# neggles/neurosis

Hardware: AMD Instinct MI355X
Metric: train images/sec (node) SDXL 1024^2 (higher is better)
Workload: dtype bf16

## Files before the change

### neurosis_amd/csrc/conv_wgrad_halo.h

```cpp
#pragma once


typedef __attribute__((address_space(3))) char* wh_lds;
typedef __attribute__((address_space(3))) short4_t* wh_lds4;

__device__ __forceinline__ int wh_swz_x(int slot) { return (((slot >> 1) & 1) << 2) | ((slot >> 2) & 3); }
__device__ __forceinline__ int wh_swz_dy(int px) { return ((px & 3) << 2) | ((px >> 2) & 3); }

__device__ __forceinline__ bf16x8_t wh_read(wh_lds lo, wh_lds hi) {
  const short4_t a = __builtin_amdgcn_ds_read_tr16_b64_v4i16((wh_lds4)lo);
  const short4_t b = __builtin_amdgcn_ds_read_tr16_b64_v4i16((wh_lds4)hi);
  short8_t r;
  r[0] = a[0]; r[1] = a[1]; r[2] = a[2]; r[3] = a[3];
  r[4] = b[0]; r[5] = b[1]; r[6] = b[2]; r[7] = b[3];
  return __builtin_bit_cast(bf16x8_t, r);
}

struct WhStager {
  int xd, xe, dd, de;
  int n, ty, tx;

  __device__ __forceinline__ void init(const NkGemmParams& p, int t, int txn, int tyn, int lane) {
    const int per_img = txn * tyn;
    n = t / per_img;
    const int rem = t - n * per_img;
    ty = rem / txn;
    tx = rem - ty * txn;
    const int l8 = lane >> 3, l16 = lane >> 4;
    xd = (lane & 7) ^ ((((l8 >> 1) & 1) << 2) | (l8 >> 2));
    xe = l8 * p.gb.C;
    dd = (lane & 15) ^ (l16 << 2);
    de = l16 * (int)p.lda;
  }
  __device__ __forceinline__ void issue(const NkGemmParams& p, char* stage, int txn, int tyn, int cb, int ib, int wave, int lane) {
    const NkGather& g = p.gb;
    const int h0 = ty * WH_TH, w0 = tx * WH_TW;
    const bf16_t* xo = p.B + (((long)n * g.H + h0 - 1) * g.W + (w0 - 1)) * g.C + ib * WH_BCI;
    const bf16_t* dyo = p.A + (((long)n * g.H + h0) * g.W + w0) * p.lda + cb * WH_BCO;
    const bf16_t* zp = (const bf16_t*)nk_zero_page;
    int l8 = lane >> 3, l16 = lane >> 4, xd_ = xd, xe_ = xe, dd_ = dd, de_ = de;
    asm volatile("" : "+v"(l8), "+v"(l16), "+v"(xd_), "+v"(xe_), "+v"(dd_), "+v"(de_));
#pragma unroll
    for (int i = 0; i < 8; ++i) {
      const int pc = wave + 8 * i;
      if (pc < 30) {
        const int hr = pc / 5, pg = pc - hr * 5;
        const bool row_ok = (unsigned)(h0 - 1 + hr) < (unsigned)g.H;
        const int slot = pg * 8 + l8;
        const bool v = row_ok && slot < WH_TW + 2 && (unsigned)(w0 - 1 + slot) < (unsigned)g.W;
        const int off = (hr * g.W + pg * 8) * g.C + xe_ + ((xd_ ^ ((pg & 1) << 1)) << 3);
        __builtin_amdgcn_global_load_lds((nk_gptr)(v ? xo + off : zp), (nk_lptr)(stage + (hr * WH_HS + pg * 8) * 128), 16, 0, 0);
      } else if (pc < 62) {
        const int q = pc - 30;
        const bool row_ok = h0 + (q >> 3) < g.H;
        const int chunk = dd_ ^ (q & 3);
        const bool v = row_ok && w0 + (q & 7) * 4 + l16 < g.W && cb * WH_BCO + chunk * 8 < p.M;
        const int off = ((q >> 3) * g.W + (q & 7) * 4) * (int)p.lda + de_ + (chunk << 3);
        __builtin_amdgcn_global_load_lds((nk_gptr)(v ? dyo + off : zp), (nk_lptr)(stage + WH_X_BYTES + q * 1024), 16, 0, 0);
      }
    }
    if (++tx == txn) { tx = 0; if (++ty == tyn) { ty = 0; ++n; } }
  }
};

template <int BIAS>
__global__ __launch_bounds__(512, 2) void nk_conv3x3_wgrad_halo_kernel(const NkGemmParams p) {
  extern __shared__ __attribute__((aligned(16))) char smem[];
  const int tid = threadIdx.x, lane = tid & 63;
  const int wave = __builtin_amdgcn_readfirstlane(tid >> 6);
  const int cs = wave & 3, is = wave >> 2;
  const NkGather& g = p.gb;
  const int Cin = g.C, Cout = p.M;
  const int nci = Cin / WH_BCI;
  const int nblk = ((Cout + WH_BCO - 1) / WH_BCO) * nci;
  const int blk = blockIdx.x % nblk, split = blockIdx.x / nblk;
  const int cb = blk / nci, ib = blk - cb * nci;
  const int txn = (g.W + WH_TW - 1) / WH_TW, tyn = (g.H + WH_TH - 1) / WH_TH;
  const int T = p.halo_nb * txn * tyn;
  const int t0 = split * p.ksplit_len, t1 = min(T, t0 + p.ksplit_len);

  float16_t acc[9];
#pragma unroll
  for (int t = 0; t < 9; ++t)
#pragma unroll
    for (int r = 0; r < 16; ++r) acc[t][r] = 0.f;
  float bsum = 0.f;

  const int h = lane >> 5, g1 = (lane >> 4) & 1, q4 = (lane & 15) >> 2, pp = lane & 3;
  unsigned xo[3][2], dyo[2];
#pragma unroll
  for (int j = 0; j < 2; ++j) {
#pragma unroll
    for (int a = 0; a < 3; ++a) {
      const int row = a + 4 * h + q4 + 8 * j;
      xo[a][j] = (unsigned)(row * 128 + (((4 * is + 2 * g1 + (pp >> 1)) ^ wh_swz_x(row)) << 4) + 8 * (pp & 1));
    }
    const int row = 4 * h + q4 + 8 * j;
    dyo[j] = (unsigned)(WH_X_BYTES + row * 256 + (((4 * cs + 2 * g1 + (pp >> 1)) ^ wh_swz_dy(row)) << 4) + 8 * (pp & 1));
  }
  const wh_lds sm = (wh_lds)smem;

  WhStager stg;
  stg.init(p, t0 < t1 ? t0 : 0, txn, tyn, lane);
  if (t0 < t1) stg.issue(p, smem, txn, tyn, cb, ib, wave, lane);
  for (int t = t0; t < t1; ++t) {
    const int st = (t - t0) & 1;
    asm volatile("s_waitcnt vmcnt(0)" ::: "memory");
    __syncthreads();
    if (t + 1 < t1) stg.issue(p, smem + (st ^ 1) * WH_STAGE, txn, tyn, cb, ib, wave, lane);
    const wh_lds base = sm + st * WH_STAGE;
#pragma unroll
    for (int kg = 0; kg < 8; ++kg) {
      const int r = kg >> 1, c = (kg & 1) * 16;
      const bf16x8_t af = wh_read(base + dyo[0] + kg * 4096, base + dyo[1] + kg * 4096);
      if constexpr (BIAS) {
        const short8_t raw = __builtin_bit_cast(short8_t, af);
#pragma unroll
        for (int e = 0; e < 8; ++e) bsum += bf2f((bf16_t)raw[e]);
      }
#pragma unroll
      for (int kh = 0; kh < 3; ++kh)
#pragma unroll
        for (int kw = 0; kw < 3; ++kw) {
          const int off = ((r + kh) * WH_HS + c) * 128;
          const bf16x8_t xf = wh_read(base + xo[kw][0] + off, base + xo[kw][1] + off);
          acc[kh * 3 + kw] = __builtin_amdgcn_mfma_f32_32x32x16_bf16(af, xf, acc[kh * 3 + kw], 0, 0, 0);
        }
    }
  }

  float* dw = (float*)p.C;
  const int ci = ib * WH_BCI + is * 32 + (lane & 31);
  const int co_base = cb * WH_BCO + cs * 32 + 4 * h;
  const bool atomic = gridDim.x > (unsigned)nblk || p.accumulate == 1;
#pragma unroll
  for (int t = 0; t < 9; ++t)
#pragma unroll
    for (int r = 0; r < 16; ++r) {
      const int co = co_base + (r & 3) + 8 * (r >> 2);
      if (co < Cout) {
        float* dst = dw + (long)co * p.ldc + t * Cin + ci;
        const float v = acc[t][r] * p.alpha;
        if (atomic) unsafeAtomicAdd(dst, v);
        else *dst = v;
      }
    }
  if constexpr (BIAS) {
    if (ib == 0 && is == 0) {
      bsum += __shfl_xor(bsum, 32);
      const int co = cb * WH_BCO + cs * 32 + (lane & 31);
      if (lane < 32 && co < Cout) {
        if (atomic) unsafeAtomicAdd(p.dbias + co, bsum * p.alpha);
        else p.dbias[co] = bsum * p.alpha;
      }
    }
  }
}
```

Baseline: 27.03.

## Spread halo wgrad DMA issue across MFMA steps and window LDS reads

Restructures the 3x3 conv weight-gradient halo kernel so that the next tile's global-to-LDS loads are issued one piece per k-group, interleaved with the MFMA work, instead of all at once after the barrier. The tile body now preloads a sliding window of input-halo fragments and dY fragments into registers, reading each halo row once rather than re-reading it for every kernel-row tap. DMA uses inline asm that sets m0 directly, and the last tile is peeled so the prefetch condition disappears from the loop. Optional timestamp instrumentation is added behind a macro. The extra register windows may raise VGPR pressure under the 512x2 launch bound.

```diff
diff --git a/neurosis_amd/csrc/conv_wgrad_halo.h b/neurosis_amd/csrc/conv_wgrad_halo.h
--- a/neurosis_amd/csrc/conv_wgrad_halo.h
+++ b/neurosis_amd/csrc/conv_wgrad_halo.h
@@ -14,6 +14,18 @@
   r[0] = a[0]; r[1] = a[1]; r[2] = a[2]; r[3] = a[3];
   r[4] = b[0]; r[5] = b[1]; r[6] = b[2]; r[7] = b[3];
   return __builtin_bit_cast(bf16x8_t, r);
+}
+
+#ifndef NK_WGH_ASM_DMA
+#define NK_WGH_ASM_DMA 1
+#endif
+__device__ __forceinline__ void wh_dma(const bf16_t* src, unsigned dst) {
+#if NK_WGH_ASM_DMA
+  unsigned keep;
+  asm volatile("s_mov_b32 %0, m0\n\ts_mov_b32 m0, %2\n\ts_nop 0\n\tglobal_load_lds_dwordx4 %1, off\n\ts_mov_b32 m0, %0" : "=&s"(keep) : "v"(src), "s"(dst) : "memory");
+#else
+  __builtin_amdgcn_global_load_lds((nk_gptr)src, (nk_lptr)(wh_lds)(unsigned long)dst, 16, 0, 0);
+#endif
 }
 
 struct WhStager {
@@ -32,36 +44,155 @@
     dd = (lane & 15) ^ (l16 << 2);
     de = l16 * (int)p.lda;
   }
-  __device__ __forceinline__ void issue(const NkGemmParams& p, char* stage, int txn, int tyn, int cb, int ib, int wave, int lane) {
+  __device__ __forceinline__ void piece(const NkGemmParams& p, unsigned stage, int cb, int ib, int wave, int lane, int i) const {
     const NkGather& g = p.gb;
     const int h0 = ty * WH_TH, w0 = tx * WH_TW;
-    const bf16_t* xo = p.B + (((long)n * g.H + h0 - 1) * g.W + (w0 - 1)) * g.C + ib * WH_BCI;
-    const bf16_t* dyo = p.A + (((long)n * g.H + h0) * g.W + w0) * p.lda + cb * WH_BCO;
     const bf16_t* zp = (const bf16_t*)nk_zero_page;
     int l8 = lane >> 3, l16 = lane >> 4, xd_ = xd, xe_ = xe, dd_ = dd, de_ = de;
-    asm volatile("" : "+v"(l8), "+v"(l16), "+v"(xd_), "+v"(xe_), "+v"(dd_), "+v"(de_));
+    if (i >= 4) {
+      asm volatile("" : "+v"(l8), "+v"(xd_), "+v"(xe_));
+      const bf16_t* xo = p.B + (((long)n * g.H + h0 - 1) * g.W + (w0 - 1)) * g.C + ib * WH_BCI;
+      const int pc = 8 * (i - 4) + (i == 7 && wave >= 6 ? wave - 2 : wave);
+      const int hr = pc / 5, pg = pc - hr * 5;
+      const bool row_ok = (unsigned)(h0 - 1 + hr) < (unsigned)g.H;
+      const int slot = pg * 8 + l8;
+      const bool v = row_ok && slot < WH_TW + 2 && (unsigned)(w0 - 1 + slot) < (unsigned)g.W;
+      const int off = (hr * g.W + pg * 8) * g.C + xe_ + ((xd_ ^ ((pg & 1) << 1)) << 3);
+      wh_dma(v ? xo + off : zp, stage + (hr * WH_HS + pg * 8) * 128);
+    } else {
+      asm volatile("" : "+v"(l16), "+v"(dd_), "+v"(de_));
+      const bf16_t* dyo = p.A + (((long)n * g.H + h0) * g.W + w0) * p.lda + cb * WH_BCO;
+      const int q = wave + 8 * i;
+      const bool row_ok = h0 + (q >> 3) < g.H;
+      const int chunk = dd_ ^ (q & 3);
+      const bool v = row_ok && w0 + (q & 7) * 4 + l16 < g.W && cb * WH_BCO + chunk * 8 < p.M;
+      const int off = ((q >> 3) * g.W + (q & 7) * 4) * (int)p.lda + de_ + (chunk << 3);
+      wh_dma(v ? dyo + off : zp, stage + WH_X_BYTES + q * 1024);
+    }
+  }
+  __device__ __forceinline__ void advance(int txn, int tyn) {
+    if (++tx == txn) { tx = 0; if (++ty == tyn) { ty = 0; ++n; } }
+  }
+  __device__ __forceinline__ void issue(const NkGemmParams& p, unsigned stage, int txn, int tyn, int cb, int ib, int wave, int lane) {
+#pragma unroll
+    for (int i = 0; i < 8; ++i) piece(p, stage, cb, ib, wave, lane, i);
+    advance(txn, tyn);
+  }
+};
+
+#ifndef NK_WGH_WINDOW
+#define NK_WGH_WINDOW 1
+#endif
+#ifndef NK_WGH_SPREAD
+#define NK_WGH_SPREAD 1
+#endif
+#ifdef NK_WGH_STAMPS
+#define WGH_SLOTS 20
+#define WGH_MAXWG 4096
+__device__ unsigned long long nk_wgh_stamp_buf[WGH_SLOTS * WGH_MAXWG];
+extern "C" int nk_debug_wgh_stamps(unsigned long long* host_out, int nwg) {
+  if (nwg < 0 || nwg > WGH_MAXWG) return 1;
+  return hipMemcpyFromSymbol(host_out, HIP_SYMBOL(nk_wgh_stamp_buf), (size_t)nwg * WGH_SLOTS * sizeof(unsigned long long)) == hipSuccess ? 0 : 1;
+}
+struct WghClock {
+  unsigned long long last;
+  unsigned sum[10];
+  __device__ __forceinline__ static unsigned long long now() {
+    unsigned long long t;
+    __builtin_amdgcn_sched_barrier(0);
+    asm volatile("s_memtime %0\n\ts_waitcnt lgkmcnt(0)" : "=s"(t) :: "memory");
+    __builtin_amdgcn_sched_barrier(0);
+    return t;
+  }
+  __device__ __forceinline__ void start() {
+#pragma unroll
+    for (int i = 0; i < 10; ++i) sum[i] = 0;
+    last = now();
+  }
+  __device__ __forceinline__ void lap(int i) { const unsigned long long t = now(); sum[i] += (unsigned)(t - last); last = t; }
+  __device__ __forceinline__ void skip() { last = now(); }
+};
+#else
+struct WghClock {
+  __device__ __forceinline__ void start() {}
+  __device__ __forceinline__ void lap(int) {}
+  __device__ __forceinline__ void skip() {}
+};
+#endif
+
+template <int BIAS, bool NEXT>
+__device__ __forceinline__ void wh_tile(float16_t (&acc)[9], float& bsum, const wh_lds base, const unsigned (&xo)[3][2], const unsigned (&dyo)[2],
+                                        const WhStager& stg, const NkGemmParams& p, unsigned nstage, int cb, int ib, int wave, int lane, WghClock& clk) {
+  if constexpr (NEXT && !NK_WGH_SPREAD) {
+#pragma unroll
+    for (int i = 0; i < 8; ++i) stg.piece(p, nstage, cb, ib, wave, lane, i);
+  }
+  clk.lap(1);
+  if constexpr (NK_WGH_WINDOW) {
+    bf16x8_t hx[2][WH_TH + 2][3];
+    bf16x8_t af[8];
+    af[0] = wh_read(base + dyo[0], base + dyo[1]);
+#pragma unroll
+    for (int hr = 0; hr < 2; ++hr)
+#pragma unroll
+      for (int kw = 0; kw < 3; ++kw) hx[0][hr][kw] = wh_read(base + xo[kw][0] + hr * WH_HS * 128, base + xo[kw][1] + hr * WH_HS * 128);
 #pragma unroll
     for (int i = 0; i < 8; ++i) {
-      const int pc = wave + 8 * i;
-      if (pc < 30) {
-        const int hr = pc / 5, pg = pc - hr * 5;
-        const bool row_ok = (unsigned)(h0 - 1 + hr) < (unsigned)g.H;
-        const int slot = pg * 8 + l8;
-        const bool v = row_ok && slot < WH_TW + 2 && (unsigned)(w0 - 1 + slot) < (unsigned)g.W;
-        const int off = (hr * g.W + pg * 8) * g.C + xe_ + ((xd_ ^ ((pg & 1) << 1)) << 3);
-        __builtin_amdgcn_global_load_lds((nk_gptr)(v ? xo + off : zp), (nk_lptr)(stage + (hr * WH_HS + pg * 8) * 128), 16, 0, 0);
-      } else if (pc < 62) {
-        const int q = pc - 30;
-        const bool row_ok = h0 + (q >> 3) < g.H;
-        const int chunk = dd_ ^ (q & 3);
-        const bool v = row_ok && w0 + (q & 7) * 4 + l16 < g.W && cb * WH_BCO + chunk * 8 < p.M;
-        const int off = ((q >> 3) * g.W + (q & 7) * 4) * (int)p.lda + de_ + (chunk << 3);
-        __builtin_amdgcn_global_load_lds((nk_gptr)(v ? dyo + off : zp), (nk_lptr)(stage + WH_X_BYTES + q * 1024), 16, 0, 0);
-      }
-    }
-    if (++tx == txn) { tx = 0; if (++ty == tyn) { ty = 0; ++n; } }
-  }
-};
+      const int ch = i >> 2, r = i & 3;
+#pragma unroll
+      for (int kw = 0; kw < 3; ++kw) {
+        const int off = ((r + 2) * WH_HS + ch * 16) * 128;
+        hx[ch][r + 2][kw] = wh_read(base + xo[kw][0] + off, base + xo[kw][1] + off);
+      }
+      if (i < 7) {
+        const int kg = 2 * ((i + 1) & 3) + ((i + 1) >> 2);
+        af[i + 1] = wh_read(base + dyo[0] + kg * 4096, base + dyo[1] + kg * 4096);
+      }
+      if (i == 3) {
+#pragma unroll
+        for (int hr = 0; hr < 2; ++hr)
+#pragma unroll
+          for (int kw = 0; kw < 3; ++kw) {
+            const int off = (hr * WH_HS + 16) * 128;
+            hx[1][hr][kw] = wh_read(base + xo[kw][0] + off, base + xo[kw][1] + off);
+          }
+      }
+      if constexpr (NEXT && NK_WGH_SPREAD) stg.piece(p, nstage, cb, ib, wave, lane, i);
+      if constexpr (BIAS) {
+        const short8_t raw = __builtin_bit_cast(short8_t, af[i]);
+#pragma unroll
+        for (int e = 0; e < 8; ++e) bsum += bf2f((bf16_t)raw[e]);
+      }
+#pragma unroll
+      for (int kh = 0; kh < 3; ++kh)
+#pragma unroll
+        for (int kw = 0; kw < 3; ++kw) acc[kh * 3 + kw] = __builtin_amdgcn_mfma_f32_32x32x16_bf16(af[i], hx[ch][r + kh][kw], acc[kh * 3 + kw], 0, 0, 0);
+      clk.lap(2 + i);
+      __builtin_amdgcn_sched_barrier(0);
+    }
+  } else {
+#pragma unroll
+    for (int kg = 0; kg < 8; ++kg) {
+      const int r = kg >> 1, c = (kg & 1) * 16;
+      const bf16x8_t af = wh_read(base + dyo[0] + kg * 4096, base + dyo[1] + kg * 4096);
+      if constexpr (NEXT && NK_WGH_SPREAD) stg.piece(p, nstage, cb, ib, wave, lane, kg);
+      if constexpr (BIAS) {
+        const short8_t raw = __builtin_bit_cast(short8_t, af);
+#pragma unroll
+        for (int e = 0; e < 8; ++e) bsum += bf2f((bf16_t)raw[e]);
+      }
+#pragma unroll
+      for (int kh = 0; kh < 3; ++kh)
+#pragma unroll
+        for (int kw = 0; kw < 3; ++kw) {
+          const int off = ((r + kh) * WH_HS + c) * 128;
+          const bf16x8_t xf = wh_read(base + xo[kw][0] + off, base + xo[kw][1] + off);
+          acc[kh * 3 + kw] = __builtin_amdgcn_mfma_f32_32x32x16_bf16(af, xf, acc[kh * 3 + kw], 0, 0, 0);
+        }
+      clk.lap(2 + kg);
+    }
+  }
+}
 
 template <int BIAS>
 __global__ __launch_bounds__(512, 2) void nk_conv3x3_wgrad_halo_kernel(const NkGemmParams p) {
@@ -78,6 +209,10 @@
   const int txn = (g.W + WH_TW - 1) / WH_TW, tyn = (g.H + WH_TH - 1) / WH_TH;
   const int T = p.halo_nb * txn * tyn;
   const int t0 = split * p.ksplit_len, t1 = min(T, t0 + p.ksplit_len);
+  WghClock clk;
+#ifdef NK_WGH_STAMPS
+  unsigned long long s_entry = WghClock::now(), s_first = s_entry, s_rt0 = 0;
+#endif
 
   float16_t acc[9];
 #pragma unroll
@@ -99,35 +234,38 @@
     dyo[j] = (unsigned)(WH_X_BYTES + row * 256 + (((4 * cs + 2 * g1 + (pp >> 1)) ^ wh_swz_dy(row)) << 4) + 8 * (pp & 1));
   }
   const wh_lds sm = (wh_lds)smem;
+  const unsigned lds0 = (unsigned)(unsigned long)sm;
 
   WhStager stg;
-  stg.init(p, t0 < t1 ? t0 : 0, txn, tyn, lane);
-  if (t0 < t1) stg.issue(p, smem, txn, tyn, cb, ib, wave, lane);
-  for (int t = t0; t < t1; ++t) {
+  stg.init(p, t0, txn, tyn, lane);
+  if (t0 >= t1) return;
+  stg.issue(p, lds0, txn, tyn, cb, ib, wave, lane);
+  clk.start();
+  for (int t = t0; t + 1 < t1; ++t) {
     const int st = (t - t0) & 1;
     asm volatile("s_waitcnt vmcnt(0)" ::: "memory");
     __syncthreads();
-    if (t + 1 < t1) stg.issue(p, smem + (st ^ 1) * WH_STAGE, txn, tyn, cb, ib, wave, lane);
-    const wh_lds base = sm + st * WH_STAGE;
-#pragma unroll
-    for (int kg = 0; kg < 8; ++kg) {
-      const int r = kg >> 1, c = (kg & 1) * 16;
-      const bf16x8_t af = wh_read(base + dyo[0] + kg * 4096, base + dyo[1] + kg * 4096);
-      if constexpr (BIAS) {
-        const short8_t raw = __builtin_bit_cast(short8_t, af);
-#pragma unroll
-        for (int e = 0; e < 8; ++e) bsum += bf2f((bf16_t)raw[e]);
-      }
-#pragma unroll
-      for (int kh = 0; kh < 3; ++kh)
-#pragma unroll
-        for (int kw = 0; kw < 3; ++kw) {
-          const int off = ((r + kh) * WH_HS + c) * 128;
-          const bf16x8_t xf = wh_read(base + xo[kw][0] + off, base + xo[kw][1] + off);
-          acc[kh * 3 + kw] = __builtin_amdgcn_mfma_f32_32x32x16_bf16(af, xf, acc[kh * 3 + kw], 0, 0, 0);
-        }
-    }
-  }
+#ifdef NK_WGH_STAMPS
+    if (t == t0) { clk.skip(); s_first = clk.last; s_rt0 = __builtin_amdgcn_s_memrealtime(); __builtin_amdgcn_s_waitcnt(0xC07F); }
+    else clk.lap(0);
+#endif
+    wh_tile<BIAS, true>(acc, bsum, sm + st * WH_STAGE, xo, dyo, stg, p, lds0 + (st ^ 1) * WH_STAGE, cb, ib, wave, lane, clk);
+    stg.advance(txn, tyn);
+  }
+  {
+    const int st = (t1 - 1 - t0) & 1;
+    asm volatile("s_waitcnt vmcnt(0)" ::: "memory");
+    __syncthreads();
+#ifdef NK_WGH_STAMPS
+    if (t1 - 1 == t0) { clk.skip(); s_first = clk.last; s_rt0 = __builtin_amdgcn_s_memrealtime(); __builtin_amdgcn_s_waitcnt(0xC07F); }
+    else clk.lap(0);
+#endif
+    wh_tile<BIAS, false>(acc, bsum, sm + st * WH_STAGE, xo, dyo, stg, p, lds0, cb, ib, wave, lane, clk);
+  }
+#ifdef NK_WGH_STAMPS
+  const unsigned long long s_loop = WghClock::now(), s_rt1 = __builtin_amdgcn_s_memrealtime();
+  __builtin_amdgcn_s_waitcnt(0xC07F);
+#endif
 
   float* dw = (float*)p.C;
   const int ci = ib * WH_BCI + is * 32 + (lane & 31);
@@ -155,4 +293,14 @@
       }
     }
   }
-}
+#ifdef NK_WGH_STAMPS
+  asm volatile("s_waitcnt vmcnt(0)" ::: "memory");
+  const unsigned long long s_end = WghClock::now();
+  if (tid == 0 && blockIdx.x < WGH_MAXWG) {
+    unsigned long long* o = nk_wgh_stamp_buf + (size_t)blockIdx.x * WGH_SLOTS;
+    o[0] = s_entry; o[1] = s_first; o[2] = s_loop; o[3] = s_end; o[4] = s_rt0; o[5] = s_rt1; o[6] = (unsigned long long)max(t1 - t0, 0);
+#pragma unroll
+    for (int i = 0; i < 10; ++i) o[7 + i] = clk.sum[i];
+  }
+#endif
+}
```

After: 27.14, median of 6. No clear change (+0.4%).
